# Daaohame/RAHT-3DGS-codec

Hardware: AMD Instinct MI355X
Metric: M-Gaussians/s fwd+inv RAHT, 59-ch SH3 3DGS (higher is better)
Workload: dtype f32 (xyz columns: f64); 1 GPU; cfg3: 2999072 Gaussians (3000000 draws/GPU, J=12, 59 channels), fwd RAHT + quantize/reorder + dequantize/un-reorder + inv RAHT (quantization fused into the transform kernels); the 3 xyz columns carried in float64 inside the same launches (raht_fwd_quant_mixed / raht_dequant_inv_mixed): the reference's integers on every column; rows_per_gpu=2999072, channels=59, depth_J=12, engine=tile, quantize=True, parallelism=1 GPU, world=1

## Files before the change

### raht-3dgs-codec_amd/csrc/plan.hip

```cpp
#include "raht_common.h"

#include <algorithm>
#include <cstdlib>
#include <cstring>
#include <exception>
#include <new>

namespace raht {

__global__ void compact_scatter_kernel(const uint32_t *in, const uint32_t *flag, const uint32_t *pos, uint32_t *out, int64_t n);

static thread_local char g_err[512] = "";

void set_error(const char *fmt, ...)
{
    va_list ap;
    va_start(ap, fmt);
    vsnprintf(g_err, sizeof(g_err), fmt, ap);
    va_end(ap);
}

int check_plan_device(const raht_plan *plan, const char *what)
{
    if (!plan) { set_error("%s: NULL plan", what); return RAHT_ERR_INVALID; }
// ... 433 lines not shown
    for (auto &st : sc.stages) {
        if (st.rows) dev_free(st.rows);
        if (st.surv_off) dev_free(st.surv_off);
        if (st.e_wl) dev_free(st.e_wl);
        if (st.e_wr) dev_free(st.e_wr);
        if (st.e_lvl) dev_free(st.e_lvl);
        if (st.e_ht) dev_free(st.e_ht);
        if (st.arrive) dev_free(st.arrive);
        if (st.e_pos) dev_free(st.e_pos);
        if (st.t_pj) dev_free(st.t_pj);
        if (st.t_ab32) dev_free(st.t_ab32);
        if (st.t_ab64) dev_free(st.t_ab64);
        if (st.t_root) dev_free(st.t_root);
        if (st.t_lev) dev_free(st.t_lev);
        if (st.ws) dev_free(st.ws);
    }
    sc.stages.clear();
}

int ensure_workspace(Schedule *sc, size_t row_bytes, bool split)
{
    if (row_bytes <= sc->ws_row_bytes && split == sc->ws_split) return RAHT_OK;
    row_bytes = std::max(row_bytes, sc->ws_row_bytes);
    for (size_t k = 1; k < sc->stages.size(); ++k) {
        Stage &st = sc->stages[k];
        if (st.ws) { (void)hipDeviceSynchronize(); dev_free(st.ws); st.ws = nullptr; }
        const size_t one = (row_bytes * (size_t)st.n_entries + 255) & ~(size_t)255;
        if (dev_malloc(&st.ws, split ? 2 * one : one) != hipSuccess) {
            set_error("workspace allocation failed (%zu bytes)", split ? 2 * one : one);
            sc->ws_row_bytes = 0;
            return RAHT_ERR_NOMEM;
        }
// ... 156 lines not shown
        if (st.is_top || st.n_entries < 1) continue;
        if (st.tile_rows > HT_MAX_ROWS) { set_error("tile heights: %d rows per tile not supported", st.tile_rows); return RAHT_ERR_UNSUPPORTED; }
        if (!st.e_ht) RAHT_HIP_CHECK(dev_malloc(&st.e_ht, (size_t)st.n_entries));
        HeightStage &h = H.st[H.n_stages++];
        h.rows = st.rows; h.wl = st.rows ? st.e_wl : plan->wl; h.wr = st.rows ? st.e_wr : plan->wr; h.lvl = st.rows ? st.e_lvl : plan->lvl;
        h.ht = st.e_ht; h.n = st.n_entries; h.R = st.tile_rows; h.first_tile = H.n_tiles;
        h.n_dev = nullptr; h.kind_dev = nullptr; h.kind_tile = 0;
        H.n_tiles += (uint32_t)st.n_tiles;
        maxR = std::max(maxR, st.tile_rows);
        any_rows = any_rows || st.rows != nullptr;
        if (H.n_stages == group) RAHT_RET(flush());
    }
    return flush();
}

__global__ void top_resolve_kernel(const uint32_t *__restrict__ rows, int64_t n, const int32_t *__restrict__ wl,
                                   const int32_t *__restrict__ wr, const uint8_t *__restrict__ lvl,
                                   const int64_t *__restrict__ wsum, int top_level, uint32_t *__restrict__ pj,
                                   double *__restrict__ ab, uint8_t *__restrict__ bucket, uint32_t *__restrict__ is_root)
{
    const int64_t e = (int64_t)blockIdx.x * blockDim.x + threadIdx.x;
    if (e >= n) return;
    const int64_t r = rows ? (int64_t)rows[e] : e;
    const int l = (int)lvl[r];
    const bool merged = (r > 0) && (l < top_level);
    is_root[e] = merged ? 0u : 1u;
    bucket[e] = merged ? (uint8_t)l : (uint8_t)63;
    uint32_t rec = 0;
    double a = 0.0, b = 0.0;
    if (merged) {
// ... 599 lines not shown
        } else {
            st.tile_rows = (k == 0) ? R0 : R1;
            st.n_tiles = ceil_div(st.n_entries, st.tile_rows);
            st.surv_off = b.surv;
            b.surv = nullptr;
            if (early_heights) { st.e_ht = b.ht; b.ht = nullptr; }
        }
        sc.stages.push_back(st);
    }
    release();
    *built = true;
    *heights_done = early_heights;
    return RAHT_OK;
}

int get_schedule(raht_plan *plan, int R0, int R1, int Rf, hipStream_t s, Schedule **out)
{
    for (auto &sc : plan->schedules)
        if (sc.tile_rows == R0 && sc.tail_rows == R1 && sc.final_rows == Rf) { *out = &sc; return RAHT_OK; }
    static const bool exact_only = getenv("RAHT_SCHEDULE_EXACT") != nullptr;
    if (!exact_only && R0 >= 64 && R1 >= 64 && Rf >= 1 && Rf <= RAHT_TOP_MAX_ROWS) {
        Schedule sc;
        sc.tile_rows = R0; sc.tail_rows = R1; sc.final_rows = Rf; sc.valid = true;
        bool built = false, heights_done = false;
        RAHT_RET(build_schedule_fast(plan, R0, R1, Rf, s, sc, &built, &heights_done));
        if (built) {
            const int rch = heights_done ? RAHT_OK : launch_stage_heights(plan, sc, s);
            if (rch != RAHT_OK) { free_schedule(sc); return rch; }
            plan->schedules.push_back(sc);
            *out = &plan->schedules.back();
            return RAHT_OK;
        }
    }
    return get_schedule_exact(plan, R0, R1, Rf, s, out);
// ... 565 lines not shown
```

### raht-3dgs-codec_amd/csrc/raht_common.h

```cpp
#pragma once

#include <hip/hip_runtime.h>
#include <stdint.h>

#include <cstdarg>
#include <cstdio>
#include <deque>
#include <exception>
#include <functional>
#include <new>
#include <vector>

#include "raht.h"

#define RAHT_WAVE 64
#define RAHT_MAX_LEVELS 64

namespace raht {

void set_error(const char *fmt, ...);

#define RAHT_HIP_CHECK(expr)                                                              \
    do {                                                                                  \
        hipError_t _e = (expr);                                                           \
// ... 106 lines not shown
    uint32_t *e_pos = nullptr;
    uint8_t *e_ht = nullptr;
    uint32_t *arrive = nullptr;
    bool is_top = false;
    uint32_t n_merges = 0;
    uint32_t *t_pj = nullptr;
    float *t_ab32 = nullptr;
    double *t_ab64 = nullptr;
    uint32_t *t_root = nullptr;
    uint32_t t_loff[65] = {0};
    uint32_t t_lev_host[2 * 64] = {0};
    uint32_t *t_lev = nullptr;
    int t_nlev = 0;
    int t_nbig = 0;
    uint32_t t_small_start = 0;
};

struct Schedule {
    int tile_rows = 0;
    int tail_rows = 0;
    int final_rows = 0;
    bool valid = false;
    std::vector<Stage> stages;
    size_t ws_row_bytes = 0;
    bool ws_split = false;
};

}

struct raht_plan {
    int device = 0;
    int64_t N = 0;
    int nbits = 0;
    int max_level = -1;
    uint64_t *keys = nullptr;
    bool keys_borrowed = false;
    uint8_t *lvl = nullptr;
    int32_t *wl = nullptr;
    int32_t *wr = nullptr;
    int64_t *wsum = nullptr;
// ... 26 lines not shown
__device__ __forceinline__ void pair_weights(int64_t i, int l, int r, const int64_t *wsum, double &w0, double &w1)
{
    if (wsum) {
        w0 = (double)(wsum[i] - wsum[i - l]);
        w1 = (double)(wsum[i + r] - wsum[i]);
    } else {
        w0 = (double)l;
        w1 = (double)r;
    }
}

int ensure_level_rows(raht_plan *plan, hipStream_t s);
int get_schedule(raht_plan *plan, int tile_rows, int tail_rows, int final_rows, hipStream_t s, Schedule **out);
void pick_tail_geometry(const raht_plan *plan, int elem_size, int D, int stage0_rows, int *tail_rows, int *tail_chunk,
                        int *final_rows);
int ensure_workspace(Schedule *sc, size_t row_bytes, bool split = false);
static inline void *stage_ws(const Stage &st, bool inverse) { return st.ws ? (void *)((char *)st.ws + (inverse ? st.ws_inv_off : 0)) : nullptr; }
int pick_tile_rows(const raht_plan *plan, int elem_size, int chunk_channels);
int pick_chunk_channels(int elem_size, int D);

size_t tile_lds_bytes(int R, int elem_size, int Dc, bool ident, bool qm);
}
```

### raht-3dgs-codec_amd/csrc/transform_mx.hip

```cpp
#include "raht_common.h"
#include "raht_device.h"
#include "tile_engine.h"

#include <algorithm>
#include <cstdlib>
#include <type_traits>

namespace raht {

#ifdef RAHT_PHASE_CLOCKS
constexpr int MX_CLK_TILES = 4096, MX_CLK_SLOTS = 12;
__device__ unsigned long long g_phase_clk_mx[MX_CLK_TILES][MX_CLK_SLOTS];
#define MX_STAMP(k) do { if (IDENT && threadIdx.x == 0 && tile_id < MX_CLK_TILES) g_phase_clk_mx[tile_id][k] = __builtin_readcyclecounter(); } while (0)
#else
#define MX_STAMP(k) do { } while (0)
#endif

constexpr int MX_MAX_WIDE = 4;
constexpr int MX_PRE_ROWS = 12;
constexpr int MX_THREADS = 512;
constexpr int MX_TOP_THREADS = 1024;
constexpr int MX_TOP_SLOTS = RAHT_TOP_MAX_ROWS / MX_TOP_THREADS;

struct StepTableMX {
    StepTable f;
    double w[MX_MAX_WIDE];
};

static size_t tile_lds_bytes_mx(int R, int NF, int nwide, bool ident)
{
    const size_t data = (size_t)R * NF * 16 + (((size_t)R * nwide * 8 + 15) & ~(size_t)15);
    const size_t meta = (size_t)R * (16 + 4 + (ident ? 0 : 4) + 4 + 1);
    const size_t surv = ((size_t)R * 2 + 15) & ~(size_t)15;
    return data + ((meta + 15) & ~(size_t)15) + 1024 + surv;
}

struct MxPtrs {
    const double *in_w;
    double *out_w;
    double *wsn_w;
    double *root_w;
};

template <bool INV, bool IDENT, int SLOTS, bool ROOTS>
__device__ __forceinline__ void tile_body_mx(const TileArgs<float> &A, const MxPtrs &P, const StepTableMX &ST, const int64_t tile_id)
{
    extern __shared__ __align__(16) unsigned char smem[];
    typedef RegChunk<float> V16;
    typedef RegChunk<double> W16;
    typedef RegChunk<int32_t> I16;
    const int R = A.R;
    const int tid0 = threadIdx.x;
    const int nthreads = blockDim.x, nwv = nthreads >> 6;
    const int nwide = A.nwide;
    const int lgw = nwide > 2 ? 2 : nwide - 1;
    const int Df = A.D;
    const int Fp = A.Dp, NF = Fp >> 2;
    const int lg = A.lg, lr = 6 - A.lg;
    const uint32_t NFm = ((1u << 20) + (uint32_t)NF - 1) / (uint32_t)NF;
    auto sync_lds = [&]() { asm volatile("s_waitcnt lgkmcnt(0)\n\ts_barrier" ::: "memory"); };
    auto wait_landed = [&]() { asm volatile("s_waitcnt vmcnt(0)" ::: "memory"); };

    size_t off = 0;
    float *ftile = (float *)smem; off += (size_t)R * Fp * 4;
    double *wd = (double *)(smem + off); off += ((size_t)R * nwide * 8 + 15) & ~(size_t)15;
    unsigned char *rec_base = smem + off;
    W16 *rec_ab = (W16 *)(smem + off); off += (size_t)R * 16;
    uint32_t *rec_pj = (uint32_t *)(smem + off); off += (size_t)R * 4;
    const int pre_rows = min(MX_PRE_ROWS, (R * 20 - 8) / (Fp * 4 + nwide * 8));
    float *spre_f = (float *)rec_base;
    double *spre_w = (double *)(rec_base + (size_t)pre_rows * Fp * 4);
    int32_t *srow = (int32_t *)(smem + off); if (!IDENT) off += (size_t)R * 4;
    int32_t *sdst = (int32_t *)(smem + off); off += (size_t)R * 4;
    uint8_t *sflag = (uint8_t *)(smem + off); off += (size_t)R;
    off = (off + 15) & ~(size_t)15;
    uint32_t *hist = (uint32_t *)(smem + off);
    uint32_t *loff = hist + 64;
    uint32_t *cursor = hist + 128;
    uint32_t *scnt = hist + 196;
    off += 1024;
    uint16_t *ssurv = (uint16_t *)(smem + off);
    off += ((size_t)R * 2 + 15) & ~(size_t)15;

    TileMeta<SLOTS> M;
    load_tile_meta<float, IDENT, true, SLOTS>(A, tile_id, tid0, nthreads, M);

    auto lane_geom = [&](int tid, int &lane, int &wid, int &g, int &c4, int &fl, int &sp, int &goff, bool &head) {
        lane = tid & 63;
        wid = __builtin_amdgcn_readfirstlane(tid >> 6);
        g = lane >> lg;
        c4 = lane & ((1 << lg) - 1);
        fl = min(c4, NF - 1);
        head = c4 == 0;
        sp = fl;
        goff = min(fl * 4, Df - 4);
    };
    float my_step[4], my_rcp[4];
    auto load_steps = [&](int place) {
        const int g0 = min(place * 4, Df - 4);
#pragma unroll
        for (int i = 0; i < 4; ++i) {
            my_step[i] = ST.f.v[ST.f.n == 1 ? 0 : g0 + i];
            my_rcp[i] = refined_rcp(my_step[i]);
        }
    };

    int tid = tid0;
    asm volatile("" : "+v"(tid));
    int lane, wid, g, c4, fl, sp, goff; bool head;
    lane_geom(tid, lane, wid, g, c4, fl, sp, goff, head);
    const int64_t e0 = tile_id * R;
    const int nt = (int)min((int64_t)R, A.n_entries - e0);
    const int64_t start_row = M.start_row, end_row = M.end_row;
    const uint32_t surv_base = (uint32_t)__builtin_amdgcn_readlane((int)M.surv_raw, 0);
    const uint32_t surv_cnt = (uint32_t)__builtin_amdgcn_readlane((int)M.surv_raw, 1) - surv_base;
    int32_t m_row[SLOTS], m_wl[SLOTS], m_wr[SLOTS], m_pos[SLOTS];
    int m_lv[SLOTS], m_ht[SLOTS];
#pragma unroll
    for (int s = 0; s < SLOTS; ++s) {
        m_row[s] = M.row[s]; m_wl[s] = M.wl[s]; m_wr[s] = M.wr[s]; m_pos[s] = M.pos[s]; m_lv[s] = M.lv[s]; m_ht[s] = M.ht[s] & 63;
    }
    if (tid < 64) hist[tid] = 0;
    MX_STAMP(0);

    auto load_linear = [&](const float *dst, int chunks, const float *src) {
        const uint32_t lds0 = (uint32_t)(uintptr_t)(__attribute__((address_space(3))) const void *)dst;
        for (int it = wid; (it << 6) < chunks; it += nwv) {
            const int c = (it << 6) + lane;
            if (c < chunks) glds16<0>(src + (uint32_t)c * 4u, lds0 + ((uint32_t)it << 10));
        }
    };
    auto load_caller_rows = [&](int rows, auto src) {
        const uint32_t lds0 = (uint32_t)(uintptr_t)(__attribute__((address_space(3))) const void *)ftile;
        const int total = rows * NF;
        for (int it = wid; (it << 6) < total; it += nwv) {
            const int c = (it << 6) + lane;
            const int jr = (int)(((uint32_t)c * NFm) >> 20), ch = c - jr * NF;
            if (c < total) glds16<1>(src(jr, (uint32_t)min(ch * 4, Df - 4)), lds0 + ((uint32_t)it << 10));
        }
    };
    auto widen_row = [&](int j, auto is_int) {
        double *row = wd + __mul24(j, nwide);
        const V16 raw = *(const V16 *)(ftile + __mul24(j, Fp));
        double d[4];
#pragma unroll
        for (int i = 0; i < 4; ++i) {
            if constexpr (decltype(is_int)::value) d[i] = i < nwide ? (double)__float_as_int(raw.v[i]) * ST.w[i] : 0.0;
            else d[i] = i < nwide ? (double)raw.v[i] : 0.0;
        }
#pragma unroll
        for (int i = 0; i < 4; ++i) if (i < nwide) row[i] = d[i];
    };

    if constexpr (!INV) {
        if constexpr (IDENT) {
            const uint32_t ldc = (uint32_t)A.ld_in;
            const float *src = A.in + e0 * (int64_t)ldc;
            load_caller_rows(nt, [&](int jr, uint32_t go) { return row_at(src, (uint32_t)jr, ldc, go); });
        } else {
            load_linear(ftile, nt * NF, A.in + e0 * (int64_t)Fp);
            load_linear((const float *)wd, (nt * nwide + 1) >> 1, (const float *)(P.in_w + e0 * (int64_t)nwide));
        }
    } else {
        const int npre = A.last_stage ? 0 : (int)min(surv_cnt, (uint32_t)pre_rows);
        load_linear(spre_f, npre * NF, (const float *)A.wsn + (int64_t)surv_base * Fp);
        load_linear((const float *)spre_w, (npre * nwide + 1) >> 1, (const float *)(P.wsn_w + (int64_t)surv_base * nwide));
    }
#pragma unroll
    for (int s = 0; s < SLOTS; ++s) {
        const int j = tid + s * nthreads;
        if (j < nt) { if (!IDENT) srow[j] = m_row[s]; if (INV) sdst[j] = m_pos[s]; }
    }
    MX_STAMP(1);
    sync_lds();
    MX_STAMP(2);

    if constexpr (INV) {
        load_caller_rows(nt, [&](int jr, uint32_t go) {
            return (const void *)row_far((const int32_t *)A.Q, (uint32_t)sdst[jr], (uint32_t)A.ldq, go); });
    }

    bool m_merged[SLOTS];
    int m_rank[SLOTS];
    const uint64_t lt = (lane == 0) ? 0ull : (~0ull >> (64 - lane));
#pragma unroll
    for (int s = 0; s < SLOTS; ++s) {
        const int j = tid + s * nthreads;
        m_merged[s] = false;
        bool surv = false;
        if (j < nt) {
            const int64_t r = m_row[s];
            m_merged[s] = (r > 0) && (m_lv[s] < A.top_level) && (r - m_wl[s] >= start_row) && (r + m_wr[s] <= end_row);
            surv = !m_merged[s];
            sflag[j] = m_merged[s] ? 1 : (A.last_stage ? 2 : 0);
            if (!INV) sdst[j] = m_pos[s] | ((m_merged[s] || (A.last_stage && !ROOTS)) ? (int32_t)0x80000000 : 0);
            if (m_merged[s]) atomicAdd(&hist[m_ht[s]], 1u);
        }
        const uint64_t bal = __ballot(surv);
        m_rank[s] = __popcll(bal & lt);
        if (lane == 0 && s * nwv + wid < 32) scnt[s * nwv + wid] = (uint32_t)__popcll(bal);
    }
    sync_lds();
    MX_STAMP(3);

    if (wid == 0) {
        const uint32_t c = hist[lane];
        uint32_t inc = c;
#pragma unroll
        for (int d = 1; d < 64; d <<= 1) {
            const uint32_t t = __shfl_up(inc, d, 64);
            if (lane >= d) inc += t;
        }
        loff[lane] = inc - c;
        cursor[lane] = inc - c;
    }
#pragma unroll
    for (int s = 0; s < SLOTS; ++s) {
        const int j = tid + s * nthreads;
        if (j < nt && !m_merged[s]) {
            uint32_t before = 0;
            for (int q = 0; q < s * nwv + wid; ++q) before += scnt[q];
            ssurv[before + (uint32_t)m_rank[s]] = (uint16_t)j;
        }
    }
    if constexpr (INV) wait_landed();
    sync_lds();
    MX_STAMP(4);
    if constexpr (INV) {
        if (!A.last_stage) {
            const uint32_t n_pre = min(surv_cnt, (uint32_t)pre_rows);
            if (c4 < NF) for (uint32_t it = wid; (it << lr) < n_pre; it += nwv) {
                const uint32_t qc = min((it << lr) + g, n_pre - 1);
                const V16 x = *(const V16 *)&spre_f[__mul24((int)qc, Fp) + fl * 4];
                *(V16 *)&ftile[__mul24((int)ssurv[qc], Fp) + fl * 4] = x;
            }
            for (uint32_t c = (uint32_t)tid; c < n_pre * (uint32_t)nwide; c += (uint32_t)nthreads) {
                const uint32_t qc = c / (uint32_t)nwide, i = c - qc * (uint32_t)nwide;
                wd[__mul24((int)ssurv[qc], nwide) + i] = spre_w[c];
            }
        } else if (ROOTS) {
            if (c4 < NF) for (uint32_t it = wid; (it << lr) < surv_cnt; it += nwv) {
                const uint32_t qc = min((it << lr) + g, surv_cnt - 1);
                const V16 x = ld_chunk<float>(A.root_buf + (int64_t)(surv_base + qc) * Df + goff);
                *(V16 *)&ftile[__mul24((int)ssurv[qc], Fp) + fl * 4] = x;
            }
            for (uint32_t c = (uint32_t)tid; c < surv_cnt * (uint32_t)nwide; c += (uint32_t)nthreads) {
                const uint32_t qc = c / (uint32_t)nwide, i = c - qc * (uint32_t)nwide;
                wd[__mul24((int)ssurv[qc], nwide) + i] = P.root_w[(int64_t)surv_base * nwide + c];
            }
        }
        sync_lds();
        load_steps(fl);
        if (A.last_stage && !ROOTS && c4 < NF) for (int it = wid; (it << lr) < nt; it += nwv) {
            const int j = (it << lr) + g;
            if (j < nt && sflag[j] == 2) {
                V16 *pr = (V16 *)&ftile[__mul24(j, Fp) + fl * 4];
                const I16 raw = *(const I16 *)pr;
                V16 x;
#pragma unroll
                for (int i = 0; i < 4; ++i)
                    x.v[i] = (head && i < nwide) ? __int_as_float(raw.v[i]) : (float)raw.v[i] * my_step[i];
                *pr = x;
            }
        }
#pragma unroll
        for (int s = 0; s < SLOTS; ++s) {
            const int j = ((tid + (nthreads >> 1)) & (nthreads - 1)) + s * nthreads;
            if (j < nt && (ROOTS ? sflag[j] == 1 : sflag[j] != 0)) widen_row(j, std::true_type());
        }
    }

#pragma unroll
    for (int s = 0; s < SLOTS; ++s) {
        const int j = tid + s * nthreads;
        if (j < nt && m_merged[s]) {
            const int64_t r = m_row[s];
            const int l = m_wl[s];
            int p;
            if (IDENT) {
                p = j - l;
            } else {
                const int32_t want = (int32_t)(r - l);
                int lo = 0, hi = j - 1;
                while (lo < hi) {
                    const int mid = (lo + hi) >> 1;
                    if (srow[mid] < want) lo = mid + 1; else hi = mid;
                }
                p = lo;
            }
            double w0, w1;
            pair_weights(r, l, m_wr[s], A.wsum, w0, w1);
            const double den = w0 + w1;
            W16 ab;
            ab.v[0] = sqrt(w0 / den);
            ab.v[1] = sqrt(w1 / den);
            const uint32_t pos = atomicAdd(&cursor[m_ht[s]], 1u);
            rec_ab[pos] = ab;
            rec_pj[pos] = (uint32_t)p | ((uint32_t)j << 16);
        }
    }
    if (INV && !A.last_stage) {
        if (c4 < NF) for (uint32_t it = wid; pre_rows + (it << lr) < surv_cnt; it += nwv) {
            const uint32_t qc = min(pre_rows + (it << lr) + g, surv_cnt - 1);
            const V16 x = ld_chunk<float>(row_at((const float *)A.wsn + (int64_t)surv_base * Fp, qc, (uint32_t)Fp, (uint32_t)(fl * 4)));
            *(V16 *)&ftile[__mul24((int)ssurv[qc], Fp) + fl * 4] = x;
        }
        for (uint32_t c = (uint32_t)(pre_rows * nwide) + (uint32_t)tid; c < surv_cnt * (uint32_t)nwide; c += (uint32_t)nthreads) {
            const uint32_t qc = c / (uint32_t)nwide, i = c - qc * (uint32_t)nwide;
            wd[__mul24((int)ssurv[qc], nwide) + i] = P.wsn_w[(int64_t)surv_base * nwide + c];
        }
    }
    if constexpr (!INV) {
        wait_landed();
        if constexpr (IDENT) {
            sync_lds();
#pragma unroll
            for (int s = 0; s < SLOTS; ++s) {
                const int j = tid + s * nthreads;
                if (j < nt) widen_row(j, std::false_type());
            }
        }
        sync_lds();
    } else {
        __syncthreads();
    }
    MX_STAMP(5);

    {
        const uint32_t stride = (uint32_t)(nwv << lr);
        const uint32_t gw = (uint32_t)lane >> lgw, cw = (uint32_t)min(lane & ((1 << lgw) - 1), nwide - 1);
        const uint32_t bw = 64u >> lgw;
        const uint32_t cf = (uint32_t)fl * 4u;
        bool chained = false;
        const int loff_v = (int)loff[lane], hist_v = (int)hist[lane];
        uint64_t mask = __ballot(hist_v > 0);
        while (mask) {
            const int l = INV ? (63 - __clzll((long long)mask)) : (__ffsll((long long)mask) - 1);
            mask &= ~(1ull << l);
            const uint32_t base = (uint32_t)__builtin_amdgcn_readlane(loff_v, l), cnt = (uint32_t)__builtin_amdgcn_readlane(hist_v, l);
            auto apply_f = [&](auto UC, uint32_t mb) {
                constexpr int U = decltype(UC)::value;
                W16 ab[U];
                uint32_t pj[U];
#pragma unroll
                for (int u = 0; u < U; ++u) { const uint32_t m = base + min(mb + u * stride + g, cnt - 1); pj[u] = rec_pj[m]; ab[u] = rec_ab[m]; }
                uint32_t ip[U], ij[U];
                V16 x0[U], x1[U];
#pragma unroll
                for (int u = 0; u < U; ++u) { ip[u] = __umul24(pj[u] & 0xffffu, (uint32_t)Fp) + cf; ij[u] = __umul24(pj[u] >> 16, (uint32_t)Fp) + cf; }
// ... 89 lines not shown
#pragma unroll
                    for (int i = 0; i < 4; ++i) { const float f = (float)w[u][i]; x[u].v[i] = (head && i < nwide) ? f : x[u].v[i]; }
                    asm volatile("" : "+v"(x[u].v[0]), "+v"(x[u].v[1]), "+v"(x[u].v[2]), "+v"(x[u].v[3]));
                    if (u == 0 || ((it + nwv) << lr) < nt)
                        st_chunk<float, true>(row_at(base, (uint32_t)j[u], (uint32_t)A.ld_out, (uint32_t)goff), x[u]);
                }
            }
        } else {
            float *bf = A.out + e0 * (int64_t)Fp;
            double *bw_ = P.out_w + e0 * (int64_t)nwide;
            for (int c = tid; c < nt * NF; c += nthreads) st_chunk<float>(bf + c * 4, *(const V16 *)&ftile[c * 4]);
            for (int c = tid; c < nt * nwide; c += nthreads) bw_[c] = wd[c];
        }
    } else {
        if (!A.last_stage || ROOTS) {
            constexpr bool to_roots = ROOTS;
            float *bf = to_roots ? A.root_buf + (int64_t)surv_base * Df : A.wsn + (int64_t)surv_base * Fp;
            double *bw_ = (to_roots ? P.root_w : P.wsn_w) + (int64_t)surv_base * nwide;
            const uint32_t ldb = (uint32_t)(to_roots ? Df : Fp), cb = (uint32_t)(to_roots ? goff : fl * 4);
            if (c4 < NF) for (uint32_t it = wid; (it << lr) < surv_cnt; it += nwv) {
                const uint32_t q = min((it << lr) + g, surv_cnt - 1);
                const V16 x = *(const V16 *)&ftile[__mul24((int)ssurv[q], Fp) + fl * 4];
                st_chunk<float>(row_at(bf, q, ldb, cb), x);
            }
            for (uint32_t c = (uint32_t)tid; c < surv_cnt * (uint32_t)nwide; c += (uint32_t)nthreads) {
                const uint32_t q = c / (uint32_t)nwide, i = c - q * (uint32_t)nwide;
                bw_[c] = wd[__mul24((int)ssurv[q], nwide) + i];
            }
        }
#pragma unroll
// ... 295 lines not shown
};

static bool mx_geometry(const raht_plan *p, int D, int nwide, MxGeom &g)
{
    if (D - 4 < nwide || D > 64 + MX_MAX_WIDE) return false;
    g.nwide = nwide;
    const int NF = (D + 3) / 4;
    g.NCp = (nwide + 1) / 2 + NF;
    g.Dp = NF * 4;
    g.lg = 0;
    while ((1 << g.lg) < NF) ++g.lg;
    int r1 = 0, dc1 = 0;
    pick_tail_geometry(p, 4, D, 512, &r1, &dc1, &g.Rf);
    const size_t budget = (size_t)42 * 1280;
    auto fit = [&](int hi, bool ident, size_t cap) {
        for (int R = hi; R >= 64; --R) if (tile_lds_bytes_mx(R, NF, nwide, ident) <= cap) return R;
        return 0;
    };
    g.R0 = p->tile_rows_override > 0 ? fit(std::min(p->tile_rows_override, TILE_MAX_SLOTS * MX_THREADS), true, (size_t)128 * 1280)
                                     : fit(512, true, budget);
    if (p->tile_rows_override > 0 && p->tile_rows_override < 64) g.R0 = 0;
    if (g.R0 == 0) return false;
    g.R1 = p->tail_rows_override > 0 ? fit(std::min(p->tail_rows_override, TILE_MAX_SLOTS * MX_THREADS), false, (size_t)128 * 1280)
                                     : fit(g.R0, false, budget);
    if (p->tail_rows_override > 0 && p->tail_rows_override < 64) g.R1 = 0;
    return g.R1 != 0;
}

static void fill_steps_mx(StepTableMX &t, const double *steps, int n_steps, int nwide)
{
    float f[MAX_STEP_CH];
// ... 83 lines not shown
        if (!A.lvl || !A.wl || !A.wr || !A.ht) bad = "plan arrays";
        else if (!A.last_stage && (!A.wsn || !A.surv_off)) bad = "survivor workspace of a non-final stage";
        else if (!A.Q || !A.inv_order) bad = "Q / inv_order";
        else if (!INV && !A.in) bad = "forward input";
        else if (INV && !A.out) bad = "inverse output";
        else if ((st.rows == nullptr) != (k == 0)) bad = "stage order";
        else if (st.tile_rows < 1 || st.tile_rows > TILE_MAX_SLOTS * MX_THREADS ||
                 (int64_t)st.tile_rows * std::max<int64_t>(io.ldc, g.Dp) * 4 >= ((int64_t)1 << 31)) bad = "tile geometry (32-bit row offsets)";
        if (bad) { set_error("mixed tile stage %d (%s): missing %s", k, INV ? "inverse" : "forward", bad); return RAHT_ERR_INVALID; }
    }
    MxPtrs P;
    P.in_w = (!INV && k >= 1) ? ws_k_w : nullptr;
    P.out_w = (INV && k >= 1) ? ws_k_w : nullptr;
    P.wsn_w = ws_n_w;
    P.root_w = A.last_stage ? p->root_buf_w : nullptr;
    const size_t lds = tile_lds_bytes_mx(st.tile_rows, g.Dp / 4, g.nwide, st.rows == nullptr);
    const unsigned nt = (unsigned)st.n_tiles;
    if (k == 0 && p->ev_before) RAHT_HIP_CHECK(hipEventRecord(p->ev_before, s));
    int rc;
    if (k == 0) rc = A.root_buf ? launch_tile_mx_slots<INV, true, true>(A, P, stp, nt, lds, s) : launch_tile_mx_slots<INV, true, false>(A, P, stp, nt, lds, s);
    else rc = A.root_buf ? launch_tile_mx_slots<INV, false, true>(A, P, stp, nt, lds, s) : launch_tile_mx_slots<INV, false, false>(A, P, stp, nt, lds, s);
    if (k == 0 && p->ev_before) RAHT_HIP_CHECK(hipEventRecord(p->ev_after, s));
    return rc;
}

static int mx_check_args(const raht_plan *p, const void *a, const void *b, int D, int64_t lda, int64_t ldb, const double *steps,
                         int n_steps, int n_wide, const char *what)
{
    if (!p || !a || !b || D < 1 || lda < D || ldb < D) { set_error("%s: bad argument", what); return RAHT_ERR_INVALID; }
    RAHT_RET(check_plan_device(p, what));
    if (n_wide < 1 || n_wide > MX_MAX_WIDE || n_wide > D) { set_error("%s: n_wide must be 1..%d (and <= D)", what, MX_MAX_WIDE); return RAHT_ERR_INVALID; }
// ... 19 lines not shown
    void *const saved = p->root_buf;
    if (saved) p->root_buf = p->root_buf_w;
    const int rc = call();
    p->root_buf = saved;
    return rc;
}

static int mx_setup(raht_plan *p, int D, int n_wide, int64_t max_ld, hipStream_t s, Schedule **sc_out, MxGeom &g)
{
    *sc_out = nullptr;
    if (p->engine == RAHT_ENGINE_LEVEL || max_ld > ((int64_t)1 << 18)) return RAHT_OK;
    if (!mx_geometry(p, D, n_wide, g)) return RAHT_OK;
    Schedule *sc = nullptr;
    RAHT_RET(get_schedule(p, g.R0, g.R1, g.Rf, s, &sc));
    if (!sc->valid) return RAHT_OK;
    RAHT_RET(ensure_workspace(sc, (size_t)g.Dp * 4 + (size_t)g.nwide * 8 + 8, p->split_ws));
    *sc_out = sc;
    return RAHT_OK;
}

static int fwd_quant_mixed_impl(const raht_plan *cp, const float *C, int64_t ldc, int D, const double *steps, int n_steps, int n_wide,
                                int32_t *Q, int64_t ldq, raht_stream_t stream)
{
    raht_plan *p = const_cast<raht_plan *>(cp);
    hipStream_t s = (hipStream_t)stream;
    RAHT_RET(mx_check_args(p, C, Q, D, ldc, ldq, steps, n_steps, n_wide, "raht_fwd_quant_mixed"));
    Schedule *sc = nullptr;
    MxGeom g;
    RAHT_RET(mx_setup(p, D, n_wide, std::max(ldc, ldq), s, &sc, g));
    if (!sc) {
// ... 102 lines not shown
```

Before: 4808 M-Gaussians/s.

## Precompute per-tile merge programs once per schedule and consume them in mixed tile kernels

Adds a one-time tile_program_kernel that, for each tile, computes the height histogram prefix, merge records (partner index, destination row) and the pair weights, and stores them in a per-stage device buffer cached with the schedule. The mixed forward/inverse tile kernels now read this precomputed program instead of loading metadata, binary-searching partners, computing sqrt weights and running an LDS histogram with atomics on every call. The LDS footprint shrinks because the metadata, histogram and prefetch buffers are removed, which may allow larger tiles or more occupancy. In exchange it adds extra global reads of the program per tile, an extra device allocation, and an event to order schedule builds across streams.

```diff
diff --git a/raht-3dgs-codec_amd/csrc/plan.hip b/raht-3dgs-codec_amd/csrc/plan.hip
--- a/raht-3dgs-codec_amd/csrc/plan.hip
+++ b/raht-3dgs-codec_amd/csrc/plan.hip
@@ -471,8 +471,10 @@
         if (st.t_root) dev_free(st.t_root);
         if (st.t_lev) dev_free(st.t_lev);
         if (st.ws) dev_free(st.ws);
+        if (st.prog) dev_free(st.prog);
     }
     sc.stages.clear();
+    if (sc.ready) { (void)hipEventDestroy(sc.ready); sc.ready = nullptr; }
 }
 
 int ensure_workspace(Schedule *sc, size_t row_bytes, bool split)
@@ -659,6 +661,141 @@
     return flush();
 }
 
+struct ProgStage {
+    const uint32_t *rows; const int32_t *wl, *wr; const uint8_t *lvl, *ht; const uint32_t *pos;
+    uint32_t *prog; int64_t n; int R; uint32_t stride, ab; int compact;
+};
+
+template <int SPL>
+__global__ __launch_bounds__(64) void tile_program_kernel(const ProgStage S, int64_t N, int top_level, const int64_t *__restrict__ wsum)
+{
+    extern __shared__ __align__(16) unsigned char pg_smem[];
+    __shared__ uint32_t s_hist[64], s_cur[64];
+    uint32_t *s_row = (uint32_t *)pg_smem;
+    const int R = S.R;
+    const int lane = threadIdx.x;
+    const int64_t e0 = (int64_t)blockIdx.x * R;
+    if (e0 >= S.n) return;
+    const uint32_t *__restrict__ rows = S.rows;
+    const int nt = (int)min((int64_t)R, S.n - e0);
+    const int64_t start_row = rows ? (int64_t)rows[e0] : e0;
+    const int64_t end_row = (e0 + R < S.n) ? (rows ? (int64_t)rows[e0 + R] : e0 + R) : N;
+    uint32_t *pg = S.prog + (size_t)blockIdx.x * S.stride;
+    uint32_t *rw = pg + 32, *rec = pg + 32 + R;
+    double *ab = (double *)(pg + S.ab);
+    int lv[SPL], ht[SPL];
+    int32_t wlv[SPL], wrv[SPL];
+    uint32_t pos[SPL];
+    int64_t r[SPL];
+#pragma unroll
+    for (int s = 0; s < SPL; ++s) {
+        const int j = lane + s * 64;
+        lv[s] = 255; wlv[s] = 0; wrv[s] = 0; r[s] = 0; ht[s] = 0; pos[s] = 0;
+        if (j < nt) {
+            r[s] = rows ? (int64_t)rows[e0 + j] : e0 + j;
+            lv[s] = (int)S.lvl[e0 + j]; wlv[s] = S.wl[e0 + j]; wrv[s] = S.wr[e0 + j];
+            ht[s] = S.ht[e0 + j] & 63; pos[s] = S.pos[e0 + j];
+        }
+    }
+    s_hist[lane] = 0;
+    if (rows) {
+#pragma unroll
+        for (int s = 0; s < SPL; ++s) { const int j = lane + s * 64; if (j < nt) s_row[j] = (uint32_t)r[s]; }
+    }
+    __syncthreads();
+    bool merged[SPL];
+    int part[SPL];
+#pragma unroll
+    for (int s = 0; s < SPL; ++s) {
+        const int j = lane + s * 64;
+        merged[s] = (j < nt) && (r[s] > 0) && (lv[s] < top_level) && (r[s] - wlv[s] >= start_row) && (r[s] + wrv[s] <= end_row);
+        part[s] = 0;
+        if (merged[s]) {
+            if (!rows) part[s] = j - wlv[s];
+            else {
+                const uint32_t want = (uint32_t)(r[s] - wlv[s]);
+                int lo = 0, hi = j - 1;
+                while (lo < hi) { const int mid = (lo + hi) >> 1; if (s_row[mid] < want) lo = mid + 1; else hi = mid; }
+                part[s] = lo;
+            }
+            atomicAdd(&s_hist[ht[s]], 1u);
+        }
+        if (j < nt) rw[j] = pos[s] | (merged[s] ? 0x80000000u : 0u);
+    }
+    __syncthreads();
+    const uint32_t c = s_hist[lane];
+    uint32_t inc = c;
+#pragma unroll
+    for (int d = 1; d < 64; d <<= 1) {
+        const uint32_t t = __shfl_up(inc, d, 64);
+        if (lane >= d) inc += t;
+    }
+    ((uint16_t *)pg)[lane] = (uint16_t)inc;
+    s_cur[lane] = inc - c;
+    const uint32_t n_merged = (uint32_t)__shfl((int)inc, 63, 64);
+    __syncthreads();
+    const uint64_t lt = (lane == 0) ? 0ull : (~0ull >> (64 - lane));
+    uint32_t n_surv = 0;
+#pragma unroll
+    for (int s = 0; s < SPL; ++s) {
+        const int j = lane + s * 64;
+        const bool surv = j < nt && !merged[s];
+        const uint64_t bal = __ballot(surv);
+        if (surv) rec[n_merged + n_surv + (uint32_t)__popcll(bal & lt)] = (uint32_t)j;
+        n_surv += (uint32_t)__popcll(bal);
+        if (merged[s]) {
+            const uint32_t k = atomicAdd(&s_cur[ht[s]], 1u);
+            if (S.compact) {
+                rec[k] = (uint32_t)j | ((uint32_t)wlv[s] << 10) | ((uint32_t)wrv[s] << 20);
+            } else {
+                double w0, w1;
+                pair_weights(r[s], wlv[s], wrv[s], wsum, w0, w1);
+                const double den = w0 + w1;
+                rec[k] = (uint32_t)part[s] | ((uint32_t)j << 16);
+                ab[2 * k] = sqrt(w0 / den);
+                ab[2 * k + 1] = sqrt(w1 / den);
+            }
+        }
+    }
+}
+
+int build_tile_programs(raht_plan *plan, Schedule *sc, hipStream_t s)
+{
+    bool built = false;
+    for (auto &st : sc->stages) {
+        if (st.is_top || st.n_entries < 1 || st.prog) continue;
+        const int R = st.tile_rows;
+        if (R > HT_MAX_ROWS || !st.e_ht) { set_error("tile programs: %d rows per tile not supported", R); return RAHT_ERR_UNSUPPORTED; }
+        ProgStage P;
+        P.rows = st.rows;
+        P.wl = st.rows ? st.e_wl : plan->wl; P.wr = st.rows ? st.e_wr : plan->wr; P.lvl = st.rows ? st.e_lvl : plan->lvl;
+        P.pos = st.rows ? st.e_pos : plan->inv_order; P.ht = st.e_ht;
+        P.n = st.n_entries; P.R = R;
+        P.compact = (st.rows == nullptr && plan->wsum == nullptr) ? 1 : 0;
+        P.ab = (uint32_t)(32 + 2 * R + 3) & ~3u;
+        P.stride = P.compact ? P.ab : P.ab + 4 * (uint32_t)R;
+        if (!P.wl || !P.wr || !P.lvl || !P.pos) { set_error("tile programs: missing plan arrays"); return RAHT_ERR_INVALID; }
+        RAHT_HIP_CHECK(dev_malloc(&st.prog, sizeof(uint32_t) * (size_t)P.stride * (size_t)st.n_tiles));
+        P.prog = st.prog;
+        const size_t lds = st.rows ? (size_t)R * 4 : 0;
+        const unsigned grid = (unsigned)st.n_tiles;
+        const int spl = (R + 63) / 64;
+        if (spl <= 3) hipLaunchKernelGGL(tile_program_kernel<3>, dim3(grid), dim3(64), lds, s, P, plan->N, plan->top_level, plan->wsum);
+        else if (spl <= 4) hipLaunchKernelGGL(tile_program_kernel<4>, dim3(grid), dim3(64), lds, s, P, plan->N, plan->top_level, plan->wsum);
+        else if (spl <= 8) hipLaunchKernelGGL(tile_program_kernel<8>, dim3(grid), dim3(64), lds, s, P, plan->N, plan->top_level, plan->wsum);
+        else hipLaunchKernelGGL(tile_program_kernel<16>, dim3(grid), dim3(64), lds, s, P, plan->N, plan->top_level, plan->wsum);
+        RAHT_HIP_CHECK(hipGetLastError());
+        st.prog_stride = P.stride; st.prog_ab = P.ab; st.prog_compact = P.compact != 0;
+        built = true;
+    }
+    if (built) {
+        if (!sc->ready) RAHT_HIP_CHECK(hipEventCreateWithFlags(&sc->ready, hipEventDisableTiming));
+        RAHT_HIP_CHECK(hipEventRecord(sc->ready, s));
+        sc->ready_on = s;
+    }
+    return RAHT_OK;
+}
+
 __global__ void top_resolve_kernel(const uint32_t *__restrict__ rows, int64_t n, const int32_t *__restrict__ wl,
                                    const int32_t *__restrict__ wr, const uint8_t *__restrict__ lvl,
                                    const int64_t *__restrict__ wsum, int top_level, uint32_t *__restrict__ pj,
@@ -1288,10 +1425,26 @@
     return RAHT_OK;
 }
 
+static int build_schedule(raht_plan *plan, int R0, int R1, int Rf, hipStream_t s, Schedule **out);
+
 int get_schedule(raht_plan *plan, int R0, int R1, int Rf, hipStream_t s, Schedule **out)
 {
     for (auto &sc : plan->schedules)
-        if (sc.tile_rows == R0 && sc.tail_rows == R1 && sc.final_rows == Rf) { *out = &sc; return RAHT_OK; }
+        if (sc.tile_rows == R0 && sc.tail_rows == R1 && sc.final_rows == Rf) {
+            if (sc.ready && sc.ready_on != s) RAHT_HIP_CHECK(hipStreamWaitEvent(s, sc.ready, 0));
+            *out = &sc;
+            return RAHT_OK;
+        }
+    RAHT_RET(build_schedule(plan, R0, R1, Rf, s, out));
+    Schedule &sc = **out;
+    if (!sc.ready) RAHT_HIP_CHECK(hipEventCreateWithFlags(&sc.ready, hipEventDisableTiming));
+    RAHT_HIP_CHECK(hipEventRecord(sc.ready, s));
+    sc.ready_on = s;
+    return RAHT_OK;
+}
+
+static int build_schedule(raht_plan *plan, int R0, int R1, int Rf, hipStream_t s, Schedule **out)
+{
     static const bool exact_only = getenv("RAHT_SCHEDULE_EXACT") != nullptr;
     if (!exact_only && R0 >= 64 && R1 >= 64 && Rf >= 1 && Rf <= RAHT_TOP_MAX_ROWS) {
         Schedule sc;
diff --git a/raht-3dgs-codec_amd/csrc/raht_common.h b/raht-3dgs-codec_amd/csrc/raht_common.h
--- a/raht-3dgs-codec_amd/csrc/raht_common.h
+++ b/raht-3dgs-codec_amd/csrc/raht_common.h
@@ -144,6 +144,10 @@
     int t_nlev = 0;
     int t_nbig = 0;
     uint32_t t_small_start = 0;
+    uint32_t *prog = nullptr;
+    uint32_t prog_stride = 0;
+    uint32_t prog_ab = 0;
+    bool prog_compact = false;
 };
 
 struct Schedule {
@@ -154,6 +158,8 @@
     std::vector<Stage> stages;
     size_t ws_row_bytes = 0;
     bool ws_split = false;
+    hipEvent_t ready = nullptr;
+    hipStream_t ready_on = nullptr;
 };
 
 }
@@ -210,6 +216,7 @@
 int get_schedule(raht_plan *plan, int tile_rows, int tail_rows, int final_rows, hipStream_t s, Schedule **out);
 void pick_tail_geometry(const raht_plan *plan, int elem_size, int D, int stage0_rows, int *tail_rows, int *tail_chunk,
                         int *final_rows);
+int build_tile_programs(raht_plan *plan, Schedule *sc, hipStream_t s);
 int ensure_workspace(Schedule *sc, size_t row_bytes, bool split = false);
 static inline void *stage_ws(const Stage &st, bool inverse) { return st.ws ? (void *)((char *)st.ws + (inverse ? st.ws_inv_off : 0)) : nullptr; }
 int pick_tile_rows(const raht_plan *plan, int elem_size, int chunk_channels);
diff --git a/raht-3dgs-codec_amd/csrc/transform_mx.hip b/raht-3dgs-codec_amd/csrc/transform_mx.hip
--- a/raht-3dgs-codec_amd/csrc/transform_mx.hip
+++ b/raht-3dgs-codec_amd/csrc/transform_mx.hip
@@ -17,7 +17,6 @@
 #endif
 
 constexpr int MX_MAX_WIDE = 4;
-constexpr int MX_PRE_ROWS = 12;
 constexpr int MX_THREADS = 512;
 constexpr int MX_TOP_THREADS = 1024;
 constexpr int MX_TOP_SLOTS = RAHT_TOP_MAX_ROWS / MX_TOP_THREADS;
@@ -27,12 +26,12 @@
     double w[MX_MAX_WIDE];
 };
 
-static size_t tile_lds_bytes_mx(int R, int NF, int nwide, bool ident)
+static size_t tile_lds_bytes_mx(int R, int NF, int nwide)
 {
     const size_t data = (size_t)R * NF * 16 + (((size_t)R * nwide * 8 + 15) & ~(size_t)15);
-    const size_t meta = (size_t)R * (16 + 4 + (ident ? 0 : 4) + 4 + 1);
+    const size_t meta = (size_t)R * (16 + 4 + 4);
     const size_t surv = ((size_t)R * 2 + 15) & ~(size_t)15;
-    return data + ((meta + 15) & ~(size_t)15) + 1024 + surv;
+    return data + meta + surv;
 }
 
 struct MxPtrs {
@@ -40,6 +39,9 @@
     double *out_w;
     double *wsn_w;
     double *root_w;
+    const uint32_t *prog;
+    uint32_t prog_stride, prog_ab;
+    int prog_compact;
 };
 
 template <bool INV, bool IDENT, int SLOTS, bool ROOTS>
@@ -64,26 +66,10 @@
     size_t off = 0;
     float *ftile = (float *)smem; off += (size_t)R * Fp * 4;
     double *wd = (double *)(smem + off); off += ((size_t)R * nwide * 8 + 15) & ~(size_t)15;
-    unsigned char *rec_base = smem + off;
     W16 *rec_ab = (W16 *)(smem + off); off += (size_t)R * 16;
     uint32_t *rec_pj = (uint32_t *)(smem + off); off += (size_t)R * 4;
-    const int pre_rows = min(MX_PRE_ROWS, (R * 20 - 8) / (Fp * 4 + nwide * 8));
-    float *spre_f = (float *)rec_base;
-    double *spre_w = (double *)(rec_base + (size_t)pre_rows * Fp * 4);
-    int32_t *srow = (int32_t *)(smem + off); if (!IDENT) off += (size_t)R * 4;
     int32_t *sdst = (int32_t *)(smem + off); off += (size_t)R * 4;
-    uint8_t *sflag = (uint8_t *)(smem + off); off += (size_t)R;
-    off = (off + 15) & ~(size_t)15;
-    uint32_t *hist = (uint32_t *)(smem + off);
-    uint32_t *loff = hist + 64;
-    uint32_t *cursor = hist + 128;
-    uint32_t *scnt = hist + 196;
-    off += 1024;
     uint16_t *ssurv = (uint16_t *)(smem + off);
-    off += ((size_t)R * 2 + 15) & ~(size_t)15;
-
-    TileMeta<SLOTS> M;
-    load_tile_meta<float, IDENT, true, SLOTS>(A, tile_id, tid0, nthreads, M);
 
     auto lane_geom = [&](int tid, int &lane, int &wid, int &g, int &c4, int &fl, int &sp, int &goff, bool &head) {
         lane = tid & 63;
@@ -111,17 +97,59 @@
     lane_geom(tid, lane, wid, g, c4, fl, sp, goff, head);
     const int64_t e0 = tile_id * R;
     const int nt = (int)min((int64_t)R, A.n_entries - e0);
-    const int64_t start_row = M.start_row, end_row = M.end_row;
-    const uint32_t surv_base = (uint32_t)__builtin_amdgcn_readlane((int)M.surv_raw, 0);
-    const uint32_t surv_cnt = (uint32_t)__builtin_amdgcn_readlane((int)M.surv_raw, 1) - surv_base;
-    int32_t m_row[SLOTS], m_wl[SLOTS], m_wr[SLOTS], m_pos[SLOTS];
-    int m_lv[SLOTS], m_ht[SLOTS];
+    MX_STAMP(0);
+
+    const uint32_t *pg = P.prog + (uint64_t)tile_id * P.prog_stride;
+    const int end_v = ((const uint16_t *)pg)[lane];
+    const int endm_v = lane ? ((const uint16_t *)pg)[lane - 1] : 0;
+    const uint32_t surv_raw = A.surv_off ? A.surv_off[tile_id + (tid0 & 1)] : 0u;
+    uint32_t m_rw[SLOTS], m_rec[SLOTS];
+    W16 m_ab[SLOTS];
 #pragma unroll
     for (int s = 0; s < SLOTS; ++s) {
-        m_row[s] = M.row[s]; m_wl[s] = M.wl[s]; m_wr[s] = M.wr[s]; m_pos[s] = M.pos[s]; m_lv[s] = M.lv[s]; m_ht[s] = M.ht[s] & 63;
-    }
-    if (tid < 64) hist[tid] = 0;
-    MX_STAMP(0);
+        const int j = tid0 + s * nthreads;
+        m_rw[s] = 0; m_rec[s] = 0; m_ab[s].v[0] = 0.0; m_ab[s].v[1] = 0.0;
+        if (j < nt) {
+            m_rw[s] = pg[32 + j];
+            m_rec[s] = pg[32 + R + j];
+            if (!P.prog_compact) m_ab[s] = ((const W16 *)(pg + P.prog_ab))[j];
+        }
+    }
+    auto fin_of = [&](uint32_t rw) { return (rw >> 31) != 0 || (A.last_stage && !ROOTS); };
+    auto write_dst = [&]() {
+#pragma unroll
+        for (int s = 0; s < SLOTS; ++s) {
+            const int j = tid0 + s * nthreads;
+            if (j < nt) sdst[j] = (int32_t)((m_rw[s] & 0x7fffffffu) | (fin_of(m_rw[s]) ? 0x80000000u : 0u));
+        }
+    };
+    auto write_survivors = [&](uint32_t n_merged) {
+#pragma unroll
+        for (int s = 0; s < SLOTS; ++s) {
+            const uint32_t k = (uint32_t)(tid0 + s * nthreads);
+            if (k >= n_merged && k < (uint32_t)nt) ssurv[k - n_merged] = (uint16_t)m_rec[s];
+        }
+    };
+    auto write_records = [&](uint32_t n_merged) {
+#pragma unroll
+        for (int s = 0; s < SLOTS; ++s) {
+            const uint32_t k = (uint32_t)(tid0 + s * nthreads);
+            if (k < n_merged) {
+                uint32_t pj = m_rec[s];
+                W16 ab = m_ab[s];
+                if (P.prog_compact) {
+                    const uint32_t j = pj & 1023u, l = (pj >> 10) & 1023u, r = (pj >> 20) & 1023u;
+                    const double w0 = (double)(int)l, w1 = (double)(int)r;
+                    const double den = w0 + w1;
+                    ab.v[0] = sqrt(w0 / den);
+                    ab.v[1] = sqrt(w1 / den);
+                    pj = (j - l) | (j << 16);
+                }
+                rec_ab[k] = ab;
+                rec_pj[k] = pj;
+            }
+        }
+    };
 
     auto load_linear = [&](const float *dst, int chunks, const float *src) {
         const uint32_t lds0 = (uint32_t)(uintptr_t)(__attribute__((address_space(3))) const void *)dst;
@@ -136,18 +164,15 @@
         for (int it = wid; (it << 6) < total; it += nwv) {
             const int c = (it << 6) + lane;
             const int jr = (int)(((uint32_t)c * NFm) >> 20), ch = c - jr * NF;
-            if (c < total) glds16<1>(src(jr, (uint32_t)min(ch * 4, Df - 4)), lds0 + ((uint32_t)it << 10));
-        }
-    };
-    auto widen_row = [&](int j, auto is_int) {
+            if (c < total) { const void *a = src(jr, (uint32_t)min(ch * 4, Df - 4)); if (a) glds16<1>(a, lds0 + ((uint32_t)it << 10)); }
+        }
+    };
+    auto widen_row = [&](int j) {
         double *row = wd + __mul24(j, nwide);
         const V16 raw = *(const V16 *)(ftile + __mul24(j, Fp));
         double d[4];
 #pragma unroll
-        for (int i = 0; i < 4; ++i) {
-            if constexpr (decltype(is_int)::value) d[i] = i < nwide ? (double)__float_as_int(raw.v[i]) * ST.w[i] : 0.0;
-            else d[i] = i < nwide ? (double)raw.v[i] : 0.0;
-        }
+        for (int i = 0; i < 4; ++i) d[i] = i < nwide ? (double)raw.v[i] : 0.0;
 #pragma unroll
         for (int i = 0; i < 4; ++i) if (i < nwide) row[i] = d[i];
     };
@@ -161,82 +186,46 @@
             load_linear(ftile, nt * NF, A.in + e0 * (int64_t)Fp);
             load_linear((const float *)wd, (nt * nwide + 1) >> 1, (const float *)(P.in_w + e0 * (int64_t)nwide));
         }
+        const uint32_t n_merged = (uint32_t)__builtin_amdgcn_readlane(end_v, 63);
+        write_dst();
+        write_survivors(n_merged);
+        write_records(n_merged);
+        MX_STAMP(1);
+        wait_landed();
+        sync_lds();
+        MX_STAMP(2);
+        if constexpr (IDENT) {
+#pragma unroll
+            for (int s = 0; s < SLOTS; ++s) {
+                const int j = tid + s * nthreads;
+                if (j < nt) widen_row(j);
+            }
+            sync_lds();
+        }
+        MX_STAMP(3);
+        MX_STAMP(4);
     } else {
-        const int npre = A.last_stage ? 0 : (int)min(surv_cnt, (uint32_t)pre_rows);
-        load_linear(spre_f, npre * NF, (const float *)A.wsn + (int64_t)surv_base * Fp);
-        load_linear((const float *)spre_w, (npre * nwide + 1) >> 1, (const float *)(P.wsn_w + (int64_t)surv_base * nwide));
-    }
-#pragma unroll
-    for (int s = 0; s < SLOTS; ++s) {
-        const int j = tid + s * nthreads;
-        if (j < nt) { if (!IDENT) srow[j] = m_row[s]; if (INV) sdst[j] = m_pos[s]; }
-    }
-    MX_STAMP(1);
-    sync_lds();
-    MX_STAMP(2);
-
-    if constexpr (INV) {
-        load_caller_rows(nt, [&](int jr, uint32_t go) {
-            return (const void *)row_far((const int32_t *)A.Q, (uint32_t)sdst[jr], (uint32_t)A.ldq, go); });
-    }
-
-    bool m_merged[SLOTS];
-    int m_rank[SLOTS];
-    const uint64_t lt = (lane == 0) ? 0ull : (~0ull >> (64 - lane));
-#pragma unroll
-    for (int s = 0; s < SLOTS; ++s) {
-        const int j = tid + s * nthreads;
-        m_merged[s] = false;
-        bool surv = false;
-        if (j < nt) {
-            const int64_t r = m_row[s];
-            m_merged[s] = (r > 0) && (m_lv[s] < A.top_level) && (r - m_wl[s] >= start_row) && (r + m_wr[s] <= end_row);
-            surv = !m_merged[s];
-            sflag[j] = m_merged[s] ? 1 : (A.last_stage ? 2 : 0);
-            if (!INV) sdst[j] = m_pos[s] | ((m_merged[s] || (A.last_stage && !ROOTS)) ? (int32_t)0x80000000 : 0);
-            if (m_merged[s]) atomicAdd(&hist[m_ht[s]], 1u);
-        }
-        const uint64_t bal = __ballot(surv);
-        m_rank[s] = __popcll(bal & lt);
-        if (lane == 0 && s * nwv + wid < 32) scnt[s * nwv + wid] = (uint32_t)__popcll(bal);
-    }
-    sync_lds();
-    MX_STAMP(3);
-
-    if (wid == 0) {
-        const uint32_t c = hist[lane];
-        uint32_t inc = c;
-#pragma unroll
-        for (int d = 1; d < 64; d <<= 1) {
-            const uint32_t t = __shfl_up(inc, d, 64);
-            if (lane >= d) inc += t;
-        }
-        loff[lane] = inc - c;
-        cursor[lane] = inc - c;
-    }
-#pragma unroll
-    for (int s = 0; s < SLOTS; ++s) {
-        const int j = tid + s * nthreads;
-        if (j < nt && !m_merged[s]) {
-            uint32_t before = 0;
-            for (int q = 0; q < s * nwv + wid; ++q) before += scnt[q];
-            ssurv[before + (uint32_t)m_rank[s]] = (uint16_t)j;
-        }
-    }
-    if constexpr (INV) wait_landed();
-    sync_lds();
-    MX_STAMP(4);
-    if constexpr (INV) {
+        const uint32_t n_merged = (uint32_t)__builtin_amdgcn_readlane(end_v, 63);
+        write_dst();
+        write_survivors(n_merged);
+        MX_STAMP(1);
+        sync_lds();
+        MX_STAMP(2);
+        load_caller_rows(nt, [&](int jr, uint32_t go) -> const void * {
+            const uint32_t d = (uint32_t)sdst[jr];
+            return (d >> 31) ? (const void *)row_far((const int32_t *)A.Q, d & 0x7fffffffu, (uint32_t)A.ldq, go) : nullptr; });
+        write_records(n_merged);
+        const uint32_t surv_base = (uint32_t)__builtin_amdgcn_readlane((int)surv_raw, 0);
+        const uint32_t surv_cnt = (uint32_t)__builtin_amdgcn_readlane((int)surv_raw, 1) - surv_base;
         if (!A.last_stage) {
-            const uint32_t n_pre = min(surv_cnt, (uint32_t)pre_rows);
-            if (c4 < NF) for (uint32_t it = wid; (it << lr) < n_pre; it += nwv) {
-                const uint32_t qc = min((it << lr) + g, n_pre - 1);
-                const V16 x = *(const V16 *)&spre_f[__mul24((int)qc, Fp) + fl * 4];
+            if (c4 < NF) for (uint32_t it = wid; (it << lr) < surv_cnt; it += nwv) {
+                const uint32_t qc = min((it << lr) + g, surv_cnt - 1);
+                const V16 x = ld_chunk<float>(row_at((const float *)A.wsn + (int64_t)surv_base * Fp, qc, (uint32_t)Fp, (uint32_t)(fl * 4)));
                 *(V16 *)&ftile[__mul24((int)ssurv[qc], Fp) + fl * 4] = x;
             }
-            for (uint32_t c = (uint32_t)tid; c < n_pre * (uint32_t)nwide; c += (uint32_t)nthreads) {
+            for (uint32_t c = (uint32_t)tid; c < surv_cnt * (uint32_t)nwide; c += (uint32_t)nthreads) {
                 const uint32_t qc = c / (uint32_t)nwide, i = c - qc * (uint32_t)nwide;
-                wd[__mul24((int)ssurv[qc], nwide) + i] = spre_w[c];
+                wd[__mul24((int)ssurv[qc], nwide) + i] = P.wsn_w[(int64_t)surv_base * nwide + c];
             }
         } else if (ROOTS) {
             if (c4 < NF) for (uint32_t it = wid; (it << lr) < surv_cnt; it += nwv) {
@@ -249,90 +238,46 @@
                 wd[__mul24((int)ssurv[qc], nwide) + i] = P.root_w[(int64_t)surv_base * nwide + c];
             }
         }
+        MX_STAMP(3);
+        wait_landed();
         sync_lds();
+        MX_STAMP(4);
         load_steps(fl);
-        if (A.last_stage && !ROOTS && c4 < NF) for (int it = wid; (it << lr) < nt; it += nwv) {
-            const int j = (it << lr) + g;
-            if (j < nt && sflag[j] == 2) {
-                V16 *pr = (V16 *)&ftile[__mul24(j, Fp) + fl * 4];
-                const I16 raw = *(const I16 *)pr;
-                V16 x;
-#pragma unroll
-                for (int i = 0; i < 4; ++i)
-                    x.v[i] = (head && i < nwide) ? __int_as_float(raw.v[i]) : (float)raw.v[i] * my_step[i];
-                *pr = x;
-            }
-        }
 #pragma unroll
         for (int s = 0; s < SLOTS; ++s) {
-            const int j = ((tid + (nthreads >> 1)) & (nthreads - 1)) + s * nthreads;
-            if (j < nt && (ROOTS ? sflag[j] == 1 : sflag[j] != 0)) widen_row(j, std::true_type());
-        }
-    }
-
-#pragma unroll
-    for (int s = 0; s < SLOTS; ++s) {
-        const int j = tid + s * nthreads;
-        if (j < nt && m_merged[s]) {
-            const int64_t r = m_row[s];
-            const int l = m_wl[s];
-            int p;
-            if (IDENT) {
-                p = j - l;
-            } else {
-                const int32_t want = (int32_t)(r - l);
-                int lo = 0, hi = j - 1;
-                while (lo < hi) {
-                    const int mid = (lo + hi) >> 1;
-                    if (srow[mid] < want) lo = mid + 1; else hi = mid;
-                }
-                p = lo;
-            }
-            double w0, w1;
-            pair_weights(r, l, m_wr[s], A.wsum, w0, w1);
-            const double den = w0 + w1;
-            W16 ab;
-            ab.v[0] = sqrt(w0 / den);
-            ab.v[1] = sqrt(w1 / den);
-            const uint32_t pos = atomicAdd(&cursor[m_ht[s]], 1u);
-            rec_ab[pos] = ab;
-            rec_pj[pos] = (uint32_t)p | ((uint32_t)j << 16);
-        }
-    }
-    if (INV && !A.last_stage) {
-        if (c4 < NF) for (uint32_t it = wid; pre_rows + (it << lr) < surv_cnt; it += nwv) {
-            const uint32_t qc = min(pre_rows + (it << lr) + g, surv_cnt - 1);
-            const V16 x = ld_chunk<float>(row_at((const float *)A.wsn + (int64_t)surv_base * Fp, qc, (uint32_t)Fp, (uint32_t)(fl * 4)));
-            *(V16 *)&ftile[__mul24((int)ssurv[qc], Fp) + fl * 4] = x;
-        }
-        for (uint32_t c = (uint32_t)(pre_rows * nwide) + (uint32_t)tid; c < surv_cnt * (uint32_t)nwide; c += (uint32_t)nthreads) {
-            const uint32_t qc = c / (uint32_t)nwide, i = c - qc * (uint32_t)nwide;
-            wd[__mul24((int)ssurv[qc], nwide) + i] = P.wsn_w[(int64_t)surv_base * nwide + c];
-        }
-    }
-    if constexpr (!INV) {
-        wait_landed();
-        if constexpr (IDENT) {
-            sync_lds();
-#pragma unroll
-            for (int s = 0; s < SLOTS; ++s) {
-                const int j = tid + s * nthreads;
-                if (j < nt) widen_row(j, std::false_type());
+            const int j = tid0 + s * nthreads;
+            if (j < nt && fin_of(m_rw[s])) {
+                double *row = wd + __mul24(j, nwide);
+                const I16 raw = *(const I16 *)(ftile + __mul24(j, Fp));
+#pragma unroll
+                for (int i = 0; i < 4; ++i) if (i < nwide) row[i] = (double)raw.v[i] * ST.w[i];
+            }
+        }
+        if (A.last_stage && !ROOTS) {
+            const uint32_t n_fin = (uint32_t)nt - n_merged;
+            if (c4 < NF) for (uint32_t it = wid; (it << lr) < n_fin; it += nwv) {
+                const uint32_t qc = (it << lr) + g;
+                if (qc < n_fin) {
+                    V16 *pr = (V16 *)&ftile[__mul24((int)ssurv[qc], Fp) + fl * 4];
+                    const I16 raw = *(const I16 *)pr;
+                    V16 x;
+#pragma unroll
+                    for (int i = 0; i < 4; ++i)
+                        x.v[i] = (head && i < nwide) ? __int_as_float(raw.v[i]) : (float)raw.v[i] * my_step[i];
+                    *pr = x;
+                }
             }
         }
         sync_lds();
-    } else {
-        __syncthreads();
     }
     MX_STAMP(5);
-
     {
         const uint32_t stride = (uint32_t)(nwv << lr);
         const uint32_t gw = (uint32_t)lane >> lgw, cw = (uint32_t)min(lane & ((1 << lgw) - 1), nwide - 1);
         const uint32_t bw = 64u >> lgw;
         const uint32_t cf = (uint32_t)fl * 4u;
         bool chained = false;
-        const int loff_v = (int)loff[lane], hist_v = (int)hist[lane];
+        const int loff_v = endm_v, hist_v = end_v - endm_v;
         uint64_t mask = __ballot(hist_v > 0);
         while (mask) {
             const int l = INV ? (63 - __clzll((long long)mask)) : (__ffsll((long long)mask) - 1);
@@ -452,6 +397,8 @@
         }
     } else {
         if (!A.last_stage || ROOTS) {
+            const uint32_t surv_base = (uint32_t)__builtin_amdgcn_readlane((int)surv_raw, 0);
+            const uint32_t surv_cnt = (uint32_t)__builtin_amdgcn_readlane((int)surv_raw, 1) - surv_base;
             constexpr bool to_roots = ROOTS;
             float *bf = to_roots ? A.root_buf + (int64_t)surv_base * Df : A.wsn + (int64_t)surv_base * Fp;
             double *bw_ = (to_roots ? P.root_w : P.wsn_w) + (int64_t)surv_base * nwide;
@@ -777,7 +724,7 @@
     pick_tail_geometry(p, 4, D, 512, &r1, &dc1, &g.Rf);
     const size_t budget = (size_t)42 * 1280;
     auto fit = [&](int hi, bool ident, size_t cap) {
-        for (int R = hi; R >= 64; --R) if (tile_lds_bytes_mx(R, NF, nwide, ident) <= cap) return R;
+        for (int R = hi; R >= 64; --R) if (tile_lds_bytes_mx(R, NF, nwide) <= cap) return R;
         return 0;
     };
     g.R0 = p->tile_rows_override > 0 ? fit(std::min(p->tile_rows_override, TILE_MAX_SLOTS * MX_THREADS), true, (size_t)128 * 1280)
@@ -891,7 +838,9 @@
     P.out_w = (INV && k >= 1) ? ws_k_w : nullptr;
     P.wsn_w = ws_n_w;
     P.root_w = A.last_stage ? p->root_buf_w : nullptr;
-    const size_t lds = tile_lds_bytes_mx(st.tile_rows, g.Dp / 4, g.nwide, st.rows == nullptr);
+    P.prog = st.prog; P.prog_stride = st.prog_stride; P.prog_ab = st.prog_ab; P.prog_compact = st.prog_compact ? 1 : 0;
+    if (!P.prog) { set_error("mixed tile stage %d: missing tile programs", k); return RAHT_ERR_INVALID; }
+    const size_t lds = tile_lds_bytes_mx(st.tile_rows, g.Dp / 4, g.nwide);
     const unsigned nt = (unsigned)st.n_tiles;
     if (k == 0 && p->ev_before) RAHT_HIP_CHECK(hipEventRecord(p->ev_before, s));
     int rc;
@@ -941,6 +890,7 @@
     Schedule *sc = nullptr;
     RAHT_RET(get_schedule(p, g.R0, g.R1, g.Rf, s, &sc));
     if (!sc->valid) return RAHT_OK;
+    RAHT_RET(build_tile_programs(p, sc, s));
     RAHT_RET(ensure_workspace(sc, (size_t)g.Dp * 4 + (size_t)g.nwide * 8 + 8, p->split_ws));
     *sc_out = sc;
     return RAHT_OK;
```

New measurement: 4986 M-Gaussians/s (median of 6 runs). 1.04x the previous value.
